# tomcreutz/slam-uwv_kalman_filters

Hardware: AMD Instinct MI355X
Metric: UKF predict+update steps/sec at batch=65536 PoseUKF instances, 1 & 8 GPU (higher is better)
Workload: dtype f64

## Files before the change

### slam-uwv_kalman_filters_amd/csrc/uwvk_psp_pair.hip

```cpp
#define PSP_PAIR 1
#define PSP_NS psp2
#ifndef PSP_PAIR_WAVES
#define PSP_PAIR_WAVES 3
#endif
#include <algorithm>
#include <atomic>

#define UWVK_POSE_KERNEL_BODIES
#include "uwvk_pose_kernels.hpp"
#include "uwvk_psp_dev.hpp"
#include "uwvk_psp.hpp"

namespace uwvk {
namespace psp2 {

UWVK_DEV int half() { return (int)(threadIdx.x >> 5) & 1; }

struct PUnit {
  int64_t unit, e0, e1, tslot;
  int chunk;
};
UWVK_DEV PUnit ticket_unit(const EpochArgs& ea, uint32_t u) {
  PUnit t{(int64_t)u, ea.first, ea.first + ea.count, 0, -1};
  if (ea.chunks > 1 && (int64_t)u >= ea.tail0) {
    const uint32_t q = u - (uint32_t)ea.tail0, m = (uint32_t)ea.r_x;
    const uint32_t k = q / m, r = q - k * m;
    t.unit = ea.tail0 + r;
    t.chunk = (int)k;
    t.tslot = r;
    t.e0 = ea.first + ea.count * k / ea.chunks;
    t.e1 = ea.first + ea.count * (k + 1) / ea.chunks;
  }
  return t;
}
UWVK_DEV uint32_t ticket_issue(const EpochArgs& ea) {
  uint32_t v = 0;
  if (lane_id() == 0) v = __hip_atomic_fetch_add(ea.ticket, 1u, __ATOMIC_RELAXED, __HIP_MEMORY_SCOPE_AGENT);
  return v;
}
UWVK_DEV uint32_t ticket_value(const EpochArgs& ea, uint32_t v) {
  return __builtin_amdgcn_readfirstlane(v) - ea.ticket_base;
}
UWVK_DEV bool tail_wait(uint32_t* f, uint32_t want, uint32_t bound) {
  uint32_t n = 0;
  if (lane_id() == 0) {
    while (__hip_atomic_load(f, __ATOMIC_RELAXED, __HIP_MEMORY_SCOPE_AGENT) != want && ++n < bound)
      __builtin_amdgcn_s_sleep(64);
  }
  n = __builtin_amdgcn_readfirstlane(n);
  __builtin_amdgcn_wave_barrier();
  __builtin_amdgcn_fence(__ATOMIC_ACQUIRE, "agent");
  return n < bound;
}
UWVK_DEV void tail_signal(const EpochArgs& ea, int64_t t, int chunk) {
  __builtin_amdgcn_fence(__ATOMIC_RELEASE, "agent");
  __builtin_amdgcn_wave_barrier();
  if (lane_id() == 0)
    __hip_atomic_store(ea.tail_flag + t, ea.tag * 16u + (uint32_t)(chunk + 1), __ATOMIC_RELAXED,
                       __HIP_MEMORY_SCOPE_AGENT);
}

UWVK_DEV int pd_pidx(int e) {
  int i = (int)((sqrtf(8.0f * (float)e + 1.0f) - 1.0f) * 0.5f);
  if (((i + 1) * (i + 2)) / 2 <= e) i++;
  if ((i * (i + 1)) / 2 > e) i--;
  const int j = e - (i * (i + 1)) / 2;
  const int I = pd_dof(i), J = pd_dof(j);
  return (I * (I + 1)) / 2 + J;
}
UWVK_DEV constexpr int pd_diag53(int t) { return ((19 + t) * (20 + t)) / 2 + 19 + t; }
constexpr int kPdTab = PG<26>::NSLOT * kLanes;
static_assert(PG<53>::NP <= 65536, "16-bit table entries");
UWVK_DEV void pd_tab_fill(unsigned short* tab, int l) {
#pragma unroll
  for (int t = 0; t < PG<26>::NSLOT; t++) {
    const int e = l + kLanes * t;
    tab[e] = (unsigned short)(e < PG<26>::NP ? pd_pidx(e) : 0);
  }
  psync();
}

UWVK_DEV void lane_proc(const PoseBufs& b, const PoseShared& sh, int64_t inst, int s, ProcCtx& pc) {
  using L = Lay<26>;
  const uwvk_pose_parameter& P = sh.p;
  pc.vpart = s < 3 ? L::s_vel + s : ((s >= L::s_vel && s < L::s_vel + 3) ? L::s_acc + s - L::s_vel : -1);
  pc.nt_lane = 0.0;
  pc.off_lane = 0.0;
  int k = -1;
  if (s >= L::s_bg && s < L::s_bg + 3) { pc.nt_lane = sh.ntau[0]; pc.off_lane = P.gyro_bias_offset[s - L::s_bg]; }
  if (s >= L::s_ba && s < L::s_ba + 3) { pc.nt_lane = sh.ntau[1]; pc.off_lane = P.acc_bias_offset[s - L::s_ba]; }
  if (s >= L::s_wv && s < L::s_wv + 4) pc.nt_lane = sh.ntau[5];
  if (s >= L::s_badcp && s < L::s_badcp + 2) pc.nt_lane = sh.ntau[6];
  if (s == L::s_rho) { k = 27; pc.nt_lane = sh.ntau[7]; }
  if (k >= 0) pc.off_lane = b.off[inst * 28 + k];
  pc.nt_tan = 0.0;
  if (s < 26 && scaled_dof(s)) pc.nt_tan = tan_ntau_sel<26>(s, sh);
}

struct ParLane {
  double q;
  double off;
  double nt;
};
UWVK_DEV ParLane par_lane(const PoseBufs& b, const PoseShared& sh, int64_t inst, int t) {
  ParLane p{0.0, 0.0, 0.0};
  if (t < kPdN) {
    p.q = reinterpret_cast<const double2*>(b.Qp)[PG<26>::NP + t].y;
    p.off = b.off[inst * 28 + t];
    p.nt = t < 9 ? sh.ntau[2] : (t < 18 ? sh.ntau[3] : sh.ntau[4]);
  }
  return p;
}
UWVK_DEV void par_epoch(double* px, int t, double dt, const ParLane& p) {
  if (t < kPdN) {
    const double a = 1.0 + dt * p.nt;
    const double v = px[t], m = px[32 + t];
    px[t] = a * (a * v) + p.q;
    px[32 + t] = m + dt * (p.nt * (m - p.off));
  }
}

UWVK_DEV void load_pair(PspSmem<26>& sm, double* px, const unsigned short* tab, const PoseBufs& b, int64_t inst,
                        int l) {
  using G = PG<26>;
  const double* gs = b.sigma + inst * (int64_t)PG<53>::NP;
  const double* gm = b.mu + inst * (int64_t)Lay<53>::store;
  double v[G::NSLOT];
#pragma unroll
  for (int t = 0; t < G::NSLOT; t++) {
    const int e = l + kLanes * t;
    v[t] = e < G::NP ? gs[tab[e]] : 0.0;
  }
  const double m = l < Lay<26>::store ? gm[pd_store(l)] : 0.0;
  const bool pl = l < kPdN;
  const double ps = pl ? gs[pd_diag53(l)] : 0.0, pm = pl ? gm[20 + l] : 0.0;
#pragma unroll
  for (int t = 0; t < G::NSLOT; t++) {
    const int e = l + kLanes * t;
    if (e < G::NP) sm.S[e] = v[t];
  }
  if (l < Lay<26>::store) sm.mu[l] = m;
  if (pl) {
    px[l] = ps;
    px[32 + l] = pm;
  }
  psync();
}
UWVK_DEV void store_pair(const PspSmem<26>& sm, const double* px, const unsigned short* tab, const PoseBufs& b,
                         int64_t inst, int l) {
  using G = PG<26>;
  double* gs = b.sigma + inst * (int64_t)PG<53>::NP;
  double* gm = b.mu + inst * (int64_t)Lay<53>::store;
  static_assert(G::NSLOT * kLanes <= G::NP + Lay<26>::store + PG<26>::STG, "slot over-read stays in PspSmem");
  double v[G::NSLOT];
#pragma unroll
  for (int t = 0; t < G::NSLOT; t++) v[t] = flat(sm)[l + kLanes * t];
  const double m = flat(sm)[kFlatMu<26> + l];
  const bool pl = l < kPdN;
  const double ps = px[l], pm = px[32 + l];
#pragma unroll
  for (int t = 0; t < G::NSLOT; t++) {
    const int e = l + kLanes * t;
    if (e < G::NP) gs[tab[e]] = v[t];
  }
  if (l < Lay<26>::store) gm[pd_store(l)] = m;
  if (pl) {
    gs[pd_diag53(l)] = ps;
    gm[20 + l] = pm;
  }
}

UWVK_DEV void load_pair26(PspSmem<26>& sm, const PoseBufs& b, int64_t inst, int l) {
  using G = PG<26>;
  const double* gs = b.sigma + inst * (int64_t)G::NP;
  const double* gm = b.mu + inst * (int64_t)Lay<26>::store;
  double v[G::NSLOT];
#pragma unroll
  for (int t = 0; t < G::NSLOT; t++) {
    const int e = l + kLanes * t;
    v[t] = e < G::NP ? gs[e] : 0.0;
  }
  const double m = l < Lay<26>::store ? gm[l] : 0.0;
#pragma unroll
  for (int t = 0; t < G::NSLOT; t++) {
    const int e = l + kLanes * t;
    if (e < G::NP) sm.S[e] = v[t];
  }
  if (l < Lay<26>::store) sm.mu[l] = m;
  psync();
}
UWVK_DEV void store_pair26(const PspSmem<26>& sm, const PoseBufs& b, int64_t inst, int l) {
  using G = PG<26>;
  double* gs = b.sigma + inst * (int64_t)G::NP;
  double* gm = b.mu + inst * (int64_t)Lay<26>::store;
  double v[G::NSLOT];
#pragma unroll
  for (int t = 0; t < G::NSLOT; t++) v[t] = flat(sm)[l + kLanes * t];
  const double m = flat(sm)[kFlatMu<26> + l];
#pragma unroll
  for (int t = 0; t < G::NSLOT; t++) {
    const int e = l + kLanes * t;
    if (e < G::NP) gs[e] = v[t];
  }
  if (l < Lay<26>::store) gm[l] = m;
}

template <int M>
UWVK_DEV void copy_zr(const double* zin, const double* Rin, double (&z)[M], double (&R)[M * M]) {
#pragma unroll
  for (int k = 0; k < M; k++) z[k] = zin[k];
#pragma unroll
  for (int k = 0; k < M * M; k++) R[k] = Rin[k];
}
UWVK_DEV bool finite_n(const double* a, int n) {
  bool ok = true;
  for (int i = 0; i < n; i++) ok = ok && __builtin_isfinite(a[i]);
  return ok;
}
UWVK_DEV const PoseShared& shared_for_epoch(const PoseBufs& b) {
  using CP = const __attribute__((address_space(4))) PoseShared*;
  CP p = (CP)b.shared;
  asm volatile("" : "+s"(p));
  return *(const PoseShared*)p;
}

template <int SR, int EVS, int PD>
__global__ __launch_bounds__(64) __attribute__((amdgpu_waves_per_eu(PSP_PAIR_WAVES, PSP_PAIR_WAVES)))
void k_psp_epoch_pair(PoseBufs b, PoseShared sh0, EpochArgs ea) {
  __shared__ PspSmemPD<26> smx[2];
  __shared__ unsigned short pdx[PD ? kPdTab : 1];
  const int h = half();
  PspSmem<26>& sm = smx[h];
  double* const px = smx[h].pS;
  constexpr int NW = PD ? 53 : 26;
  const int64_t B = b.batch;
  const uint32_t grid = gridDim.x;
  uint32_t u = blockIdx.x;
  if constexpr (PD) pd_tab_fill(pdx, olane());
#pragma unroll 1
  while (u < ea.units) {
    const PUnit tu = ticket_unit(ea, u);
    if (tu.chunk > 0 && !tail_wait(ea.tail_flag + tu.tslot, ea.tag * 16u + (uint32_t)tu.chunk, ea.wait_bound)) {
      if ((threadIdx.x & 31) == 0) {
        __hip_atomic_fetch_or(b.status + 2 * tu.unit + h, UWVK_ST_SCHEDULE, __ATOMIC_RELAXED, __HIP_MEMORY_SCOPE_AGENT);
        __hip_atomic_store(ea.fault, 1u, __ATOMIC_RELAXED, __HIP_MEMORY_SCOPE_SYSTEM);
      }
      u = grid + ticket_value(ea, ticket_issue(ea));
      psync();
      continue;
    }
    const int l = olane();
    const int64_t inst = 2 * tu.unit + h;
    const int64_t e_begin = tu.e0, e_end = tu.e1;
    bool ok = true, nan = false;
    uint32_t cnt[4] = {0, 0, 0, 0};
    ProcCtx pc;
    for (int k = 0; k < 3; k++) pc.w[k] = b.rot[inst * 3 + k];
    {
      double dtv = ea.dt;
      asm volatile("" : "+v"(dtv));
      pc.dt = dtv;
    }
    pc.off = nullptr;
    lane_proc(b, *b.shared, inst, l, pc);
    const ParLane pl = PD ? par_lane(b, *b.shared, inst, l) : ParLane{0.0, 0.0, 0.0};
    const LaneQ lq = lane_q<26, 0>(b.Qp, l);
    uint32_t fl_n = 0;
    double g_n[3] = {0, 0, 0}, a_n[3] = {0, 0, 0};
    auto fetch = [&](int64_t e) {
      fl_n = ea.flags[e];
#pragma unroll
      for (int k = 0; k < 3; k++) {
        g_n[k] = ea.gyro[(e * B + inst) * 3 + k];
        a_n[k] = ea.acc[(e * B + inst) * 3 + k];
      }
    };
    if (e_end > e_begin) fetch(e_begin);
    if constexpr (PD) load_pair(sm, px, pdx, b, inst, l);
    else load_pair26(sm, b, inst, l);
    double ds = 1.0, ids = 1.0;
    if (tu.chunk > 0) {
      const double2 c = reinterpret_cast<const double2*>(ea.tail_carry)[tu.tslot * 64 + lane_id()];
      ds = c.x;
      ids = c.y;
    }
    uint32_t vn = ticket_issue(ea);
#pragma unroll 1
    for (int64_t e = e_begin; e < e_end; e++) {
      const uint32_t fl = fl_n;
      const double g[3] = {g_n[0], g_n[1], g_n[2]}, za[3] = {a_n[0], a_n[1], a_n[2]};
      if (e + 1 < e_end) fetch(e + 1);
      if (finite_n(g, 3)) {
        for (int k = 0; k < 3; k++) pc.w[k] = g[k];
      } else {
        nan = true;
      }
      const PoseShared& sh = shared_for_epoch(b);
      if (((e - ea.first) & 1023) == 1023) psp_fold<26, 0>(sm, ds, ids);
      bool sok = psp_predict<26, 1, SR, PD>(sm, sh, pc, b.Q, b.Qp, ds, ids, lq, nullptr, px);
      if constexpr (PD) par_epoch(px, l, pc.dt, pl);
      ok = ok && sok;
      if (fl & UWVK_EV_ACC) {
        if (finite_n(za, 3)) {
          double z[3], R[9];
          copy_zr<3>(za, sh.log_acc_cov, z, R);
          psp_update<26, SR, PAcc<26>, NW>(sm, z, R, 0, PAcc<26>{}, &sok, ds, ids);
          ok = ok && sok;
        } else {
          nan = true;
        }
      }
      if (fl & UWVK_EV_DVL) {
        const double* zp = ea.dvl + ((int64_t)ea.dvl_index[e] * B + inst) * 3;
        if (finite_n(zp, 3)) {
          double z[3], R[9];
          copy_zr<3>(zp, sh.log_dvl_cov, z, R);
          cnt[0] += psp_update<26, SR, PVel<26>, NW>(sm, z, R, 0, PVel<26>{}, &sok, ds, ids);
          ok = ok && sok;
        } else {
          nan = true;
        }
      }
      if constexpr (EVS == 0) {
        if (fl & UWVK_EV_ADCP) {
          for (int c = 0; c < ea.cells; c++) {
            const double* zp = ea.adcp + (((int64_t)ea.a_index[e] * ea.cells + c) * B + inst) * 2;
            if (!finite_n(zp, 2)) {
              nan = true;
              continue;
            }
            double z[2] = {zp[0], zp[1]}, R[4] = {ea.adcp_cov[0], ea.adcp_cov[1], ea.adcp_cov[2], ea.adcp_cov[3]};
            PWater<26> hw;
            hw.cw = ea.cw[c];
            cnt[2] += psp_update<26, SR, PWater<26>, NW>(sm, z, R, 1, hw, &sok, ds, ids);
            ok = ok && sok;
          }
        }
      }
    }
    if (l == 0) {
      const uint32_t bits = (ok ? 0u : UWVK_ST_NOTPD) | (nan ? UWVK_ST_NAN : 0u);
      if (bits) __hip_atomic_fetch_or(b.status + inst, bits, __ATOMIC_RELAXED, __HIP_MEMORY_SCOPE_AGENT);
      if (e_end > e_begin) {
        b.rot[inst * 3] = pc.w[0]; b.rot[inst * 3 + 1] = pc.w[1]; b.rot[inst * 3 + 2] = pc.w[2];
      }
      if (ea.accept_counts)
        for (int k = 0; k < 4; k++) ea.accept_counts[inst * 4 + k] += cnt[k];
    }
    const uint32_t un = grid + ticket_value(ea, vn);
    const PUnit tn = ticket_unit(ea, u);
    const bool hand = tn.chunk >= 0 && tn.chunk + 1 < ea.chunks;
    if (hand) {
      double* c = ea.tail_carry + (tn.tslot * 64 + lane_id()) * 2;
      c[0] = ds;
      c[1] = ids;
      psync();
    } else {
      psp_fold<26, 0>(sm, ds, ids);
    }
    if constexpr (PD) store_pair(sm, px, pdx, b, inst, l);
    else store_pair26(sm, b, inst, l);
    if (hand) tail_signal(ea, tn.tslot, tn.chunk);
    u = un;
    psync();
  }
}

}

template <int SR, int PD>
static hipError_t launch_pair_sr(hipStream_t st, const PoseBufs& b, const PoseShared& sh, const EpochArgs& ea,
                                 int64_t grid, uint32_t ev_any) {
  const dim3 g((unsigned)grid), t(64);
  if (ev_any & UWVK_EV_PRESSURE) return hipErrorInvalidValue;
  if (ev_any & UWVK_EV_ADCP) hipLaunchKernelGGL((psp2::k_psp_epoch_pair<SR, 0, PD>), g, t, 0, st, b, sh, ea);
  else hipLaunchKernelGGL((psp2::k_psp_epoch_pair<SR, 1, PD>), g, t, 0, st, b, sh, ea);
  return hipGetLastError();
}

hipError_t launch_psp_epoch_pair(hipStream_t st, const PoseBufs& b, const PoseShared& sh, const EpochArgs& ea,
                                 int64_t grid, uint32_t ev_any, int pd) {
  if (!sh.q_simple || !ea.ticket || grid <= 0) return hipErrorInvalidValue;
  if (pd) return sh.so3_right ? launch_pair_sr<1, 1>(st, b, sh, ea, grid, ev_any)
                              : launch_pair_sr<0, 1>(st, b, sh, ea, grid, ev_any);
  return sh.so3_right ? launch_pair_sr<1, 0>(st, b, sh, ea, grid, ev_any)
                      : launch_pair_sr<0, 0>(st, b, sh, ea, grid, ev_any);
}

int64_t psp_pair_slots(int device) {
  int per_cu = 0, cus = 0;
  if (hipOccupancyMaxActiveBlocksPerMultiprocessor(&per_cu, (const void*)psp2::k_psp_epoch_pair<1, 1, 1>, 64, 0) !=
          hipSuccess ||
      hipDeviceGetAttribute(&cus, hipDeviceAttributeMultiprocessorCount, device) != hipSuccess)
    return 0;
  return (int64_t)per_cu * cus;
}

}
```

Before: 433.3 million.

## Prefetch next work unit's state into registers and hoist lane constants

```diff
diff --git a/slam-uwv_kalman_filters_amd/csrc/uwvk_psp_pair.hip b/slam-uwv_kalman_filters_amd/csrc/uwvk_psp_pair.hip
--- a/slam-uwv_kalman_filters_amd/csrc/uwvk_psp_pair.hip
+++ b/slam-uwv_kalman_filters_amd/csrc/uwvk_psp_pair.hip
@@ -2,6 +2,12 @@
 #define PSP_NS psp2
 #ifndef PSP_PAIR_WAVES
 #define PSP_PAIR_WAVES 3
+#endif
+#ifndef PSP_PAIR_HOIST
+#define PSP_PAIR_HOIST 1
+#endif
+#ifndef PSP_PAIR_PREFETCH
+#define PSP_PAIR_PREFETCH 1
 #endif
 #include <algorithm>
 #include <atomic>
@@ -80,19 +86,17 @@
   psync();
 }
 
-UWVK_DEV void lane_proc(const PoseBufs& b, const PoseShared& sh, int64_t inst, int s, ProcCtx& pc) {
+UWVK_DEV void lane_proc(const PoseShared& sh, int s, ProcCtx& pc) {
   using L = Lay<26>;
   const uwvk_pose_parameter& P = sh.p;
   pc.vpart = s < 3 ? L::s_vel + s : ((s >= L::s_vel && s < L::s_vel + 3) ? L::s_acc + s - L::s_vel : -1);
   pc.nt_lane = 0.0;
   pc.off_lane = 0.0;
-  int k = -1;
   if (s >= L::s_bg && s < L::s_bg + 3) { pc.nt_lane = sh.ntau[0]; pc.off_lane = P.gyro_bias_offset[s - L::s_bg]; }
   if (s >= L::s_ba && s < L::s_ba + 3) { pc.nt_lane = sh.ntau[1]; pc.off_lane = P.acc_bias_offset[s - L::s_ba]; }
   if (s >= L::s_wv && s < L::s_wv + 4) pc.nt_lane = sh.ntau[5];
   if (s >= L::s_badcp && s < L::s_badcp + 2) pc.nt_lane = sh.ntau[6];
-  if (s == L::s_rho) { k = 27; pc.nt_lane = sh.ntau[7]; }
-  if (k >= 0) pc.off_lane = b.off[inst * 28 + k];
+  if (s == L::s_rho) pc.nt_lane = sh.ntau[7];
   pc.nt_tan = 0.0;
   if (s < 26 && scaled_dof(s)) pc.nt_tan = tan_ntau_sel<26>(s, sh);
 }
@@ -102,11 +106,10 @@
   double off;
   double nt;
 };
-UWVK_DEV ParLane par_lane(const PoseBufs& b, const PoseShared& sh, int64_t inst, int t) {
+UWVK_DEV ParLane par_lane(const PoseBufs& b, const PoseShared& sh, int t) {
   ParLane p{0.0, 0.0, 0.0};
   if (t < kPdN) {
     p.q = reinterpret_cast<const double2*>(b.Qp)[PG<26>::NP + t].y;
-    p.off = b.off[inst * 28 + t];
     p.nt = t < 9 ? sh.ntau[2] : (t < 18 ? sh.ntau[3] : sh.ntau[4]);
   }
   return p;
@@ -120,29 +123,56 @@
   }
 }
 
-UWVK_DEV void load_pair(PspSmem<26>& sm, double* px, const unsigned short* tab, const PoseBufs& b, int64_t inst,
-                        int l) {
+struct UnitIn {
+  double v[PG<26>::NSLOT];
+  double m, ps, pm;
+  double w[3];
+  double off_rho, off_par;
+  double g[3], a[3];
+  uint32_t fl;
+  bool have;
+};
+template <int PD>
+UWVK_DEV void unit_fetch(UnitIn& in, bool have, const unsigned short* tab, const PoseBufs& b, const EpochArgs& ea,
+                         int64_t unit, int64_t e0, bool imu, int h, int l) {
   using G = PG<26>;
-  const double* gs = b.sigma + inst * (int64_t)PG<53>::NP;
-  const double* gm = b.mu + inst * (int64_t)Lay<53>::store;
-  double v[G::NSLOT];
+  const int64_t inst = have ? 2 * unit + h : 0;
+  const double* gs = b.sigma + inst * (int64_t)(PD ? PG<53>::NP : G::NP);
+  const double* gm = b.mu + inst * (int64_t)(PD ? Lay<53>::store : Lay<26>::store);
+  in.have = have;
 #pragma unroll
   for (int t = 0; t < G::NSLOT; t++) {
     const int e = l + kLanes * t;
-    v[t] = e < G::NP ? gs[tab[e]] : 0.0;
-  }
-  const double m = l < Lay<26>::store ? gm[pd_store(l)] : 0.0;
-  const bool pl = l < kPdN;
-  const double ps = pl ? gs[pd_diag53(l)] : 0.0, pm = pl ? gm[20 + l] : 0.0;
+    in.v[t] = (have && e < G::NP) ? gs[PD ? (int)tab[e] : e] : 0.0;
+  }
+  in.m = (have && l < Lay<26>::store) ? gm[PD ? pd_store(l) : l] : 0.0;
+  const bool pl = PD && have && l < kPdN;
+  in.ps = pl ? gs[pd_diag53(l)] : 0.0;
+  in.pm = pl ? gm[20 + l] : 0.0;
+  in.off_par = pl ? b.off[inst * 28 + l] : 0.0;
+  in.off_rho = (have && l == Lay<26>::s_rho) ? b.off[inst * 28 + 27] : 0.0;
+  in.fl = (have && imu) ? ea.flags[e0] : 0u;
+#pragma unroll
+  for (int k = 0; k < 3; k++) {
+    in.w[k] = have ? b.rot[inst * 3 + k] : 0.0;
+    in.g[k] = (have && imu) ? ea.gyro[(e0 * b.batch + inst) * 3 + k] : 0.0;
+    in.a[k] = (have && imu) ? ea.acc[(e0 * b.batch + inst) * 3 + k] : 0.0;
+  }
+}
+template <int PD>
+UWVK_DEV void unit_put(PspSmem<26>& sm, double* px, const UnitIn& in, int l) {
+  using G = PG<26>;
 #pragma unroll
   for (int t = 0; t < G::NSLOT; t++) {
     const int e = l + kLanes * t;
-    if (e < G::NP) sm.S[e] = v[t];
-  }
-  if (l < Lay<26>::store) sm.mu[l] = m;
-  if (pl) {
-    px[l] = ps;
-    px[32 + l] = pm;
+    if (e < G::NP) sm.S[e] = in.v[t];
+  }
+  if (l < Lay<26>::store) sm.mu[l] = in.m;
+  if constexpr (PD) {
+    if (l < kPdN) {
+      px[l] = in.ps;
+      px[32 + l] = in.pm;
+    }
   }
   psync();
 }
@@ -170,25 +200,6 @@
   }
 }
 
-UWVK_DEV void load_pair26(PspSmem<26>& sm, const PoseBufs& b, int64_t inst, int l) {
-  using G = PG<26>;
-  const double* gs = b.sigma + inst * (int64_t)G::NP;
-  const double* gm = b.mu + inst * (int64_t)Lay<26>::store;
-  double v[G::NSLOT];
-#pragma unroll
-  for (int t = 0; t < G::NSLOT; t++) {
-    const int e = l + kLanes * t;
-    v[t] = e < G::NP ? gs[e] : 0.0;
-  }
-  const double m = l < Lay<26>::store ? gm[l] : 0.0;
-#pragma unroll
-  for (int t = 0; t < G::NSLOT; t++) {
-    const int e = l + kLanes * t;
-    if (e < G::NP) sm.S[e] = v[t];
-  }
-  if (l < Lay<26>::store) sm.mu[l] = m;
-  psync();
-}
 UWVK_DEV void store_pair26(const PspSmem<26>& sm, const PoseBufs& b, int64_t inst, int l) {
   using G = PG<26>;
   double* gs = b.sigma + inst * (int64_t)G::NP;
@@ -237,6 +248,21 @@
   const uint32_t grid = gridDim.x;
   uint32_t u = blockIdx.x;
   if constexpr (PD) pd_tab_fill(pdx, olane());
+  auto lane_consts = [&](int l, ProcCtx& pc, ParLane& pl, LaneQ& lq) {
+    double dtv = ea.dt;
+    asm volatile("" : "+v"(dtv));
+    pc.dt = dtv;
+    pc.off = nullptr;
+    lane_proc(*b.shared, l, pc);
+    pl = PD ? par_lane(b, *b.shared, l) : ParLane{0.0, 0.0, 0.0};
+    lq = lane_q<26, 0>(b.Qp, l);
+  };
+  ProcCtx pc;
+  ParLane pl;
+  LaneQ lq;
+  if constexpr (PSP_PAIR_HOIST) lane_consts(olane(), pc, pl, lq);
+  UnitIn in;
+  unit_fetch<PD>(in, false, pdx, b, ea, 0, 0, false, h, 0);
 #pragma unroll 1
   while (u < ea.units) {
     const PUnit tu = ticket_unit(ea, u);
@@ -246,6 +272,7 @@
         __hip_atomic_store(ea.fault, 1u, __ATOMIC_RELAXED, __HIP_MEMORY_SCOPE_SYSTEM);
       }
       u = grid + ticket_value(ea, ticket_issue(ea));
+      in.have = false;
       psync();
       continue;
     }
@@ -254,19 +281,13 @@
     const int64_t e_begin = tu.e0, e_end = tu.e1;
     bool ok = true, nan = false;
     uint32_t cnt[4] = {0, 0, 0, 0};
-    ProcCtx pc;
-    for (int k = 0; k < 3; k++) pc.w[k] = b.rot[inst * 3 + k];
-    {
-      double dtv = ea.dt;
-      asm volatile("" : "+v"(dtv));
-      pc.dt = dtv;
-    }
-    pc.off = nullptr;
-    lane_proc(b, *b.shared, inst, l, pc);
-    const ParLane pl = PD ? par_lane(b, *b.shared, inst, l) : ParLane{0.0, 0.0, 0.0};
-    const LaneQ lq = lane_q<26, 0>(b.Qp, l);
-    uint32_t fl_n = 0;
-    double g_n[3] = {0, 0, 0}, a_n[3] = {0, 0, 0};
+    if constexpr (!PSP_PAIR_HOIST) lane_consts(l, pc, pl, lq);
+    if (!in.have) unit_fetch<PD>(in, true, pdx, b, ea, tu.unit, e_begin, e_end > e_begin, h, l);
+    for (int k = 0; k < 3; k++) pc.w[k] = in.w[k];
+    if (l == Lay<26>::s_rho) pc.off_lane = in.off_rho;
+    pl.off = in.off_par;
+    uint32_t fl_n = in.fl;
+    double g_n[3] = {in.g[0], in.g[1], in.g[2]}, a_n[3] = {in.a[0], in.a[1], in.a[2]};
     auto fetch = [&](int64_t e) {
       fl_n = ea.flags[e];
 #pragma unroll
@@ -275,9 +296,7 @@
         a_n[k] = ea.acc[(e * B + inst) * 3 + k];
       }
     };
-    if (e_end > e_begin) fetch(e_begin);
-    if constexpr (PD) load_pair(sm, px, pdx, b, inst, l);
-    else load_pair26(sm, b, inst, l);
+    unit_put<PD>(sm, px, in, l);
     double ds = 1.0, ids = 1.0;
     if (tu.chunk > 0) {
       const double2 c = reinterpret_cast<const double2*>(ea.tail_carry)[tu.tslot * 64 + lane_id()];
@@ -338,6 +357,12 @@
         }
       }
     }
+    const uint32_t un = grid + ticket_value(ea, vn);
+    {
+      const PUnit tx = ticket_unit(ea, un < ea.units ? un : 0u);
+      const bool have = PSP_PAIR_PREFETCH && un < ea.units && tx.chunk < 0;
+      unit_fetch<PD>(in, have, pdx, b, ea, tx.unit, tx.e0, tx.e1 > tx.e0, h, l);
+    }
     if (l == 0) {
       const uint32_t bits = (ok ? 0u : UWVK_ST_NOTPD) | (nan ? UWVK_ST_NAN : 0u);
       if (bits) __hip_atomic_fetch_or(b.status + inst, bits, __ATOMIC_RELAXED, __HIP_MEMORY_SCOPE_AGENT);
@@ -347,7 +372,6 @@
       if (ea.accept_counts)
         for (int k = 0; k < 4; k++) ea.accept_counts[inst * 4 + k] += cnt[k];
     }
-    const uint32_t un = grid + ticket_value(ea, vn);
     const PUnit tn = ticket_unit(ea, u);
     const bool hand = tn.chunk >= 0 && tn.chunk + 1 < ea.chunks;
     if (hand) {
```

New measurement: 442.9 million, median of 6. +2.2%, better.
